# genglongling/EE274_ConvexCaldera_LLM_quantization

Hardware: AMD Instinct MI355X
Metric: weight matrices/sec (4096x4096, rank-128, Q=2-bit) + Frob err vs ref (higher is better)
Workload: dtype f32 (fp16 W in; fp32-grade split-fp16 MFMA products, fp64 small solves; int2 codes)

## Files before the change

### ee274_convexcaldera_llm_quantization_amd/_lib.py

```python
from __future__ import annotations

import contextlib
import ctypes
import os
import threading

import torch

from . import scratch

_HERE = os.path.dirname(os.path.abspath(__file__))
LIB_PATH = os.path.join(_HERE, "libcaldera_hip.so")

CQ_F32, CQ_F16, CQ_BF16, CQ_F64 = 0, 1, 2, 3
EPI_LINEAR, EPI_RESID, EPI_WERR = 0, 1, 2
CQ_EINVAL, CQ_EHIP, CQ_EWORKSPACE = -1, -2, -3

c_i64, c_int, c_float, c_double, c_size, c_vp = (ctypes.c_int64, ctypes.c_int, ctypes.c_float,
                                                 ctypes.c_double, ctypes.c_size_t, ctypes.c_void_p)


class GemmArgs(ctypes.Structure):
    _fields_ = [
        ("M", c_i64), ("N", c_i64), ("K", c_i64), ("batch", c_i64),
# ... 686 lines not shown
    M = MA if M is None else M
    N = Bh.shape[1]
    assert lda is None or (a_blocked and lda == MA and M <= MA)
    assert Bh.shape[2] == Kd and (C is None or C.shape == (Bt, M, N))
    for t in (Ah, Al, Bh, Bl, C, P, D, out_h, out_l):
        assert t is None or t.is_contiguous()
    for t in (out_h, out_l):
        assert t is None or t.numel() >= Bt * M * N, "gemm_x3: split output buffer too small"
    g = X3Args()
    g.M, g.N, g.K, g.batch = M, N, Kd, Bt
    g.Ah, g.Al, g.lda, g.stride_a = Ah.data_ptr(), Al.data_ptr(), (MA if a_blocked else Kd), MA * Kd
    g.Bh, g.Bl, g.ldb, g.stride_b = Bh.data_ptr(), (Bl.data_ptr() if Bl is not None else None), (
        N if b_blocked else Kd), N * Kd
    g.inv_scale = inv_scale.data_ptr()
    g.C, g.ldc, g.stride_c = (C.data_ptr() if C is not None else None), N, M * N
    if P is not None:
        g.P, g.ldp, g.stride_p = P.data_ptr(), N, M * N
    if D is not None:
        g.D, g.ldd, g.stride_d = D.data_ptr(), N, M * N
    g.alpha_v = alpha_v.data_ptr() if alpha_v is not None else None
    g.beta_v = beta_v.data_ptr() if beta_v is not None else None
    g.gamma_v = gamma_v.data_ptr() if gamma_v is not None else None
    if out_h is not None and sym_bound is None:
        g.out_h, g.out_l, g.ldo, g.stride_o = out_h.data_ptr(), out_l.data_ptr(), N, M * N
        g.out_scale = out_scale
        g.overflow = overflow.data_ptr()
    g.tri = int(bool(tri))
    g.b_blocked = int(b_blocked)
    g.active = active.data_ptr() if active is not None else None
    g.a_blocked = int(a_blocked)
    g.o_blocked = int(bool(o_blocked))
    g.single = int(bool(single))
    g.b_exact = int(bool(b_exact))
    if colw is not None:
        assert colw.dtype == torch.float32 and colw.is_contiguous() and colw.shape[-1] == N
        g.colw, g.stride_colw = colw.data_ptr(), _wst(colw, Bt)
    if absmax_out is not None:
        assert absmax_out.numel() == Bt and absmax_out.element_size() == 4 and absmax_out.is_contiguous()
        absmax_out.zero_()
        g.absmax_out = absmax_out.data_ptr()
    if Ct is not None:
        _require_hip(Ct)
        assert C is not None and not tri and Ct.dtype == torch.float32 and Ct.is_contiguous() and Ct.shape == (Bt, N, M)
        g.Ct, g.stride_ct = Ct.data_ptr(), N * M
    tiles = -(-N // 384) * -(-M // 192) * Bt
    splittable = not tri and sym_bound is None and C is not None and N % 4 == 0
    if ksplit is None and not auto_split_k():
        ksplit = 1
    if ksplit is None:
        ks = min(Kd // 32 // 8, -(-512 // tiles)) if splittable and tiles < 256 and Kd >= 512 else 1
    else:
        ks = int(ksplit)
        assert ks == 1 or (splittable and ks <= Kd // 32), "gemm_x3: split-K not possible here"
    if ks > 1:
        g.ksplit = ks
        g.split_ws = scratch.get_flat("gemm_x3.split", ks * Bt * M * N, torch.float32, Ah.device).data_ptr()
    if sym_bound is not None:
        g.sym_out = 1
        g.out_bound, g.scale_out, g.inv_out = sym_bound.data_ptr(), scale_out.data_ptr(), inv_out.data_ptr()
        g.out_h, g.out_l, g.ldo, g.stride_o = out_h.data_ptr(), out_l.data_ptr(), N, M * N
        g.out_scale = out_scale
    _check(load().cq_gemm_x3(ctypes.byref(g), _stream(Ah.device)), "cq_gemm_x3")
    return C


def q_update_x3(W: torch.Tensor, L: torch.Tensor | None, R: torch.Tensor | None, bits: int, *, eps: float = 1e-8,
                codes=None, packed=None, scale=None, err_w=None, err_out=None, events=None, absmax_in=None,
                scale_hint=None, fallback_out=None):
    _require_hip(W, L, R, codes, packed, scale, err_w, err_out, scale_hint, fallback_out)
# ... 214 lines not shown
```

### ee274_convexcaldera_llm_quantization_amd/csrc/cq_x3.hip

```cpp
#include <type_traits>
#include <numeric>

#include "cq_x3.h"

namespace cq {

__device__ __forceinline__ float sym_split_scale(double bound) {
    int e = 0;
    if (bound > 0.0 && isfinite(bound)) frexp(bound, &e);
    return ldexpf(1.f, 14 - e);
}

constexpr int XG_BK = 32;

__device__ __forceinline__ int xg_swz(int row) { return (0x78 >> (2 * ((row >> 2) & 3))) & 3; }

__device__ __forceinline__ f16x8g xg_frag(const _Float16* img, int row, int chunk) {
    const int pc = chunk ^ xg_swz(row);
    return *reinterpret_cast<const f16x8g*>(img + row * XG_BK + pc * 8);
}

constexpr int XW_BM = 192, XW_BN = 384, XW_BK = 32;
constexpr int XW_THREADS = 768;
constexpr int XW_APART = XW_BM * XW_BK, XW_BPART = XW_BN * XW_BK;
// ... 467 lines not shown
                    for (int r = 0; r < 4; ++r)
                        if (col + r >= row && col + r < a.N) { Oh[o + r] = h[r]; Ol[o + r] = l[r]; }
                }
#pragma unroll
                for (int r = 0; r < 4; ++r) {
                    const int64_t c = col + r;
                    if (c > row && c < a.N) {
                        const int64_t om = (row >> 5) * (M * 32) + c * 32 + (row & 31);
                        Oh[om] = h[r];
                        Ol[om] = l[r];
                    }
                }
            }
        }
        return;
    }
    const float al_ = !live ? 0.f : a.alpha_v ? a.alpha_v[b] : 1.f;
    const float be_ = !live ? 0.f : a.beta_v ? a.beta_v[b] : 0.f;
    const float ga_ = !live ? 1.f : a.gamma_v ? a.gamma_v[b] : 0.f;
    bool ovf = false;
    uint32_t amx = 0u;
    auto al16 = [](const void* p) { return (reinterpret_cast<uintptr_t>(p) & 15) == 0; };
    auto al8 = [](const void* p) { return (reinterpret_cast<uintptr_t>(p) & 7) == 0; };
    const bool vec = (a.N & 3) == 0 && (a.ldc & 3) == 0 && (a.sc & 3) == 0 && al16(a.C) &&
                     (!a.P || ((a.ldp & 3) == 0 && (a.sp & 3) == 0 && al16(a.P))) &&
                     (!a.D || ((a.ldd & 3) == 0 && (a.sd & 3) == 0 && al16(a.D))) &&
                     (!a.Oh || ((a.o_blocked || (a.ldo & 3) == 0) && (a.so & 3) == 0 && al8(a.Oh) && al8(a.Ol)));
#pragma unroll
    for (int i = 0; i < 6; ++i) {
        const int64_t row = m0 + 96 * wm + 16 * i + l16;
        if (row >= a.M) continue;
#pragma unroll
        for (int j = 0; j < 4; ++j) {
            const int64_t col = n0 + 64 * wn + 16 * j + 4 * lq;
            if (col >= a.N) continue;
            float v[4];
#pragma unroll
            for (int r = 0; r < 4; ++r) v[r] = al_ * (acc[i][j][r] * sc);
            if (a.colw) {
                const float* cw = a.colw + b * a.scolw;
#pragma unroll
                for (int r = 0; r < 4; ++r)
                    if (col + r < a.N) v[r] *= cw[col + r];
            }
            if (vec) {
                if (a.P && be_ != 0.f) {
                    const float4 pv = *reinterpret_cast<const float4*>(a.P + b * a.sp + row * a.ldp + col);
                    v[0] += be_ * pv.x; v[1] += be_ * pv.y; v[2] += be_ * pv.z; v[3] += be_ * pv.w;
                }
                if (a.D && ga_ != 0.f) {
                    const float4 dv = *reinterpret_cast<const float4*>(a.D + b * a.sd + row * a.ldd + col);
                    v[0] += ga_ * dv.x; v[1] += ga_ * dv.y; v[2] += ga_ * dv.z; v[3] += ga_ * dv.w;
                }
                *reinterpret_cast<float4*>(a.C + b * a.sc + row * a.ldc + col) = make_float4(v[0], v[1], v[2], v[3]);
                if (a.Ct) {
#pragma unroll
                    for (int r = 0; r < 4; ++r) a.Ct[b * a.sct + (col + r) * a.M + row] = v[r];
                }
                if (a.absmax_out)
                    amx = max(amx, max(max(abs_bits(v[0]), abs_bits(v[1])), max(abs_bits(v[2]), abs_bits(v[3]))));
                if (a.Oh) {
                    _Float16 h[4], l[4];
#pragma unroll
                    for (int r = 0; r < 4; ++r) {
                        const float hs = v[r] * a.out_scale;
                        h[r] = (_Float16)hs;
                        l[r] = (_Float16)(hs - (float)h[r]);
                        ovf |= !(fabsf(hs) < 65504.f);
                    }
                    const int64_t o = b * a.so + (a.o_blocked ? (col >> 5) * (a.M * 32) + row * 32 + (col & 31)
                                                              : row * a.ldo + col);
                    *reinterpret_cast<uint2*>(a.Oh + o) = *reinterpret_cast<const uint2*>(h);
                    *reinterpret_cast<uint2*>(a.Ol + o) = *reinterpret_cast<const uint2*>(l);
                }
            } else {
#pragma unroll
                for (int r = 0; r < 4; ++r) {
                    const int64_t c = col + r;
                    if (c >= a.N) continue;
                    float w = v[r];
                    if (a.P && be_ != 0.f) w += be_ * a.P[b * a.sp + row * a.ldp + c];
                    if (a.D && ga_ != 0.f) w += ga_ * a.D[b * a.sd + row * a.ldd + c];
                    a.C[b * a.sc + row * a.ldc + c] = w;
                    if (a.Ct) a.Ct[b * a.sct + c * a.M + row] = w;
                    amx = max(amx, abs_bits(w));
                    if (a.Oh) {
                        const float hs = w * a.out_scale;
                        const _Float16 h = (_Float16)hs;
                        const int64_t o = b * a.so + (a.o_blocked ? (c >> 5) * (a.M * 32) + row * 32 + (c & 31)
                                                                  : row * a.ldo + c);
                        a.Oh[o] = h;
                        a.Ol[o] = (_Float16)(hs - (float)h);
                        ovf |= !(fabsf(hs) < 65504.f);
                    }
                }
            }
        }
    }
    if (ovf) atomicOr(a.overflow + b, 1);
    if (a.absmax_out) {
        amx = wave_max_u32(amx);
        if (lane == 0 && amx) atomicMax(a.absmax_out + b, amx);
    }
}


constexpr int XS_BM = 256, XS_BN = 256, XS_THREADS = 512;
constexpr int XS_APART = XS_BM * XW_BK, XS_BPART = XS_BN * XW_BK;
constexpr int XS_STAGE = 2 * XS_APART + 2 * XS_BPART;
constexpr size_t XS_LDS_BYTES = (size_t)2 * XS_STAGE * sizeof(_Float16);
constexpr int XS_PER_WAVE = (2 * XS_BM / 16 + 2 * XS_BN / 16) / (XS_THREADS / 64);
static_assert(XS_PER_WAVE == 8, "load split");

__device__ __forceinline__ void xs_plan(const X3K& a, int64_t m0, int64_t n0, int wid, int lane,
                                        uint32_t (&off)[XS_PER_WAVE]) {
// ... 98 lines not shown
    const int64_t nq = a.N / 4;
    const int64_t t = (int64_t)blockIdx.x * 256 + threadIdx.x;
    const int64_t b = blockIdx.y;
    const bool in = t < a.M * nq;
    uint32_t amx = 0u;
    if (in) {
    const int64_t row = t / nq, col = 4 * (t % nq);
    const bool live = !a.active || a.active[b];
    const float al_ = !live ? 0.f : a.alpha_v ? a.alpha_v[b] : 1.f;
    const float be_ = !live ? 0.f : a.beta_v ? a.beta_v[b] : 0.f;
    const float ga_ = !live ? 1.f : a.gamma_v ? a.gamma_v[b] : 0.f;
    float s[4] = {0.f, 0.f, 0.f, 0.f};
    for (int ks = 0; ks < a.ksplit; ++ks) {
        const float4 pv = *reinterpret_cast<const float4*>(a.part + ((ks * a.batch + b) * a.M + row) * a.N + col);
        s[0] += pv.x; s[1] += pv.y; s[2] += pv.z; s[3] += pv.w;
    }
    bool ovf = false;
#pragma unroll
    for (int r = 0; r < 4; ++r) {
        float w = al_ * s[r];
        if (a.colw) w *= a.colw[b * a.scolw + col + r];
        if (a.P && be_ != 0.f) w += be_ * a.P[b * a.sp + row * a.ldp + col + r];
        if (a.D && ga_ != 0.f) w += ga_ * a.D[b * a.sd + row * a.ldd + col + r];
        a.C[b * a.sc + row * a.ldc + col + r] = w;
        if (a.Ct) a.Ct[b * a.sct + (col + r) * a.M + row] = w;
        amx = max(amx, abs_bits(w));
        if (a.Oh) {
            const float hs = w * a.out_scale;
            const _Float16 h = (_Float16)hs;
            const int64_t c = col + r;
            const int64_t o = b * a.so + (a.o_blocked ? (c >> 5) * (a.M * 32) + row * 32 + (c & 31) : row * a.ldo + c);
            a.Oh[o] = h;
            a.Ol[o] = (_Float16)(hs - (float)h);
            ovf |= !(fabsf(hs) < 65504.f);
        }
    }
    if (ovf) atomicOr(a.overflow + b, 1);
    }
    if (a.absmax_out) {
        amx = wave_max_u32(amx);
        if ((threadIdx.x & 63) == 0 && amx) atomicMax(a.absmax_out + b, amx);
    }
}


template <int PASS, int BITS>
__global__ __launch_bounds__(XW_THREADS, 1) void q_update_x3_kernel(QUK q) {
    extern __shared__ __attribute__((aligned(16))) char qu_smem_raw[];
    _Float16* smem = reinterpret_cast<_Float16*>(qu_smem_raw);
    const X3K& a = q.x;
    const int64_t tiles = a.tiles_n * a.tiles_m;
    const int64_t total = tiles * a.batch;
    const int64_t orig = blockIdx.x;
    const int64_t qq = total / 8, r8 = total % 8, xcd = orig % 8;
    const int64_t lin = (xcd < r8 ? xcd * (qq + 1) : r8 * (qq + 1) + (xcd - r8) * qq) + orig / 8;
    const int64_t tile = lin % tiles;
// ... 723 lines not shown
#pragma unroll
        for (int u = 0; u < 2; ++u) {
            const int i = il + 32 * u;
            const int64_t orow = c0 + i, ocol = r0 + 8 * g;
            if (orow >= cols || ocol >= rows) continue;
            float v[8];
#pragma unroll
            for (int q = 0; q < 8; ++q) v[q] = tile[8 * g + q][i];
            if (Y) {
                float* yp = Y + ob + orow * rows + ocol;
                *reinterpret_cast<float4*>(yp) = make_float4(v[0], v[1], v[2], v[3]);
                *reinterpret_cast<float4*>(yp + 4) = make_float4(v[4], v[5], v[6], v[7]);
            }
            if (hi) {
                _Float16 h[8], l[8];
#pragma unroll
                for (int q = 0; q < 8; ++q) {
                    const float xs = v[q] * s;
                    h[q] = (_Float16)xs;
                    l[q] = (_Float16)(xs - (float)h[q]);
                }
                const int64_t o = blocked ? ob + (ocol >> 5) * cols * 32 + orow * 32 + (ocol & 31) : ob + orow * rows + ocol;
                *reinterpret_cast<uint4*>(hi + o) = *reinterpret_cast<const uint4*>(h);
                *reinterpret_cast<uint4*>(lo + o) = *reinterpret_cast<const uint4*>(l);
            }
        }
        return;
    }
    for (int i = ty; i < 64; i += 4) {
        const int64_t r = r0 + i, c = c0 + tx;
        tile[i][tx] = (r < rows && c < cols) ? Xb[r * cols + c] : 0.f;
    }
    __syncthreads();
    for (int i = ty; i < 64; i += 4) {
        const int64_t orow = c0 + i, ocol = r0 + tx;
        if (orow < cols && ocol < rows) {
            const float v = tile[tx][i];
            if (Y) Y[ob + orow * rows + ocol] = v;
            if (hi) {
                const float xs = v * s;
                const _Float16 h = (_Float16)xs;
                const int64_t o = blocked ? ob + (ocol >> 5) * cols * 32 + orow * 32 + (ocol & 31) : ob + orow * rows + ocol;
                hi[o] = h;
                lo[o] = (_Float16)(xs - (float)h);
            }
        }
    }
}


}

using namespace cq;

extern "C" {

int cq_sym_split_f16(const float* G, int64_t n, int64_t batch, int upper_only, int blocked, float x_scale,
                     uint16_t* Gh, uint16_t* Gl, float* scale_out, float* inv_scale_out, void* stream) {
    CQ_REQUIRE(G && Gh && Gl && scale_out && inv_scale_out, "cq_sym_split_f16: null pointer");
    CQ_REQUIRE(n > 0 && batch > 0 && (n * n) % 4 == 0, "cq_sym_split_f16: bad shape");
    CQ_REQUIRE(x_scale > 0.f, "cq_sym_split_f16: x_scale must be > 0");
    hipStream_t s = as_stream(stream);
    sym_scale_kernel<<<(unsigned)batch, 256, 0, s>>>(G, n, n, n * n, x_scale, scale_out, inv_scale_out);
    CQ_REQUIRE(!blocked || n % 32 == 0, "cq_sym_split_f16: blocked layout needs n % 32 == 0");
    if (upper_only || blocked) {
        CQ_REQUIRE(batch < 65536, "cq_sym_split_f16: batch too large");
        const unsigned t64 = (unsigned)ceil_div(n, 64);
// ... 31 lines not shown
int cq_split_f16(const float* X, int64_t n_per, int64_t batch, const float* scale_v, float scale, uint16_t* hi,
                 uint16_t* lo, int64_t blocked_ncols, void* stream) {
    CQ_REQUIRE(X && hi && lo, "cq_split_f16: null pointer");
    CQ_REQUIRE(n_per > 0 && batch > 0 && n_per % 4 == 0, "cq_split_f16: n_per must be a positive multiple of 4");
    CQ_REQUIRE(blocked_ncols == 0 || (blocked_ncols % 32 == 0 && n_per % blocked_ncols == 0),
               "cq_split_f16: blocked layout needs ncols % 32 == 0 dividing n_per");
    const int64_t tot4 = batch * n_per / 4;
    const unsigned grid = (unsigned)std::min<int64_t>(ceil_div(tot4, 256), 8192);
    if (blocked_ncols) {
        const int64_t rows = n_per / blocked_ncols;
        CQ_REQUIRE(batch < 65536, "cq_split_f16: batch too large");
        split_blocked_kernel<<<dim3((unsigned)ceil_div(rows, 4), (unsigned)batch), 256, 0, as_stream(stream)>>>(
            X, rows, blocked_ncols, scale_v, scale, reinterpret_cast<_Float16*>(hi), reinterpret_cast<_Float16*>(lo));
        return check_launch("cq_split_f16");
    }
    split_kernel<<<grid, 256, 0, as_stream(stream)>>>(X, n_per, scale_v, scale, reinterpret_cast<_Float16*>(hi),
                                                      reinterpret_cast<_Float16*>(lo), batch);
    return check_launch("cq_split_f16");
}

int cq_transpose_split(const float* X, int64_t rows, int64_t cols, int64_t batch, float* Y, uint16_t* hi,
                       uint16_t* lo, float scale, const float* scale_v, int blocked, void* stream) {
    CQ_REQUIRE(!blocked || rows % 32 == 0, "cq_transpose_split: blocked halves need rows % 32 == 0");
    CQ_REQUIRE(X && (Y || (hi && lo)), "cq_transpose_split: null pointer");
    CQ_REQUIRE(!hi == !lo, "cq_transpose_split: hi and lo go together");
    CQ_REQUIRE(rows > 0 && cols > 0 && batch > 0 && batch < 65536, "cq_transpose_split: bad shape");
    dim3 grid((unsigned)ceil_div(cols, 64), (unsigned)ceil_div(rows, 64), (unsigned)batch);
    auto al16 = [](const void* p) { return (reinterpret_cast<uintptr_t>(p) & 15) == 0; };
    const bool vec = rows % 8 == 0 && cols % 4 == 0 && al16(X) && (!Y || al16(Y)) && (!hi || (al16(hi) && al16(lo)));
    if (vec)
        transpose_split_kernel<true><<<grid, 256, 0, as_stream(stream)>>>(
            X, rows, cols, Y, reinterpret_cast<_Float16*>(hi), reinterpret_cast<_Float16*>(lo), scale, scale_v, blocked);
    else
        transpose_split_kernel<false><<<grid, 256, 0, as_stream(stream)>>>(
            X, rows, cols, Y, reinterpret_cast<_Float16*>(hi), reinterpret_cast<_Float16*>(lo), scale, scale_v, blocked);
    return check_launch("cq_transpose_split");
}


static int64_t qu_tiles(int64_t m, int64_t n) {
    return std::max(ceil_div(n, XW_BM) * ceil_div(m, XW_BN), ceil_div(m, XW_BM) * ceil_div(n, XW_BN));
}

static size_t qu_cand_geom(int64_t m, int64_t n, int64_t batch, int rpw, int nw, int64_t* regions_out,
                           int64_t* cap_out, int64_t* capa_out = nullptr) {
    const int64_t regions = ceil_div(m, (int64_t)rpw * nw) * nw, groups = (int64_t)rpw * n / 8;
    const bool big = m * n >= QP_BIG_NUMEL;
    const int64_t cap = ceil_div(groups * (big ? QP_CAPB_PERMILLE_BIG : QP_CAPB_PERMILLE_SMALL), (int64_t)1000);
    const int64_t capa = ceil_div(groups * (big ? QP_CAPA_PERMILLE_BIG : QP_CAPA_PERMILLE_SMALL), (int64_t)1000);
    if (regions_out) *regions_out = regions;
    if (cap_out) *cap_out = cap;
    if (capa_out) *capa_out = capa;
// ... 192 lines not shown
    const int64_t gy = std::max<int64_t>(1, std::min<int64_t>(m / 32, 16));
    dim3 grid((unsigned)(n / 64), (unsigned)gy, (unsigned)batch);
    hipStream_t s = as_stream(stream);
    double* part = sq_out ? reinterpret_cast<double*>(ws) : nullptr;
    auto h = [](uint16_t* p) { return reinterpret_cast<_Float16*>(p); };
#define CQ_RS(DT, B) residual_split_kernel<DT, B><<<grid, 256, 0, s>>>(Ws, packed, qscale, ycol, wmax, ycol_max, m, n, \
        res_out, Y_out, h(hi), h(lo), h(thi), h(tlo), scale_out, part, ycol_hi, ycol_hi_max, scale_hi_out, \
        ycol_stride, ycol_max_v, ycol_hi_max_v)
    const int bsel = packed ? bits : 2;
    if (dtype == CQ_F16) {
        switch (bsel) { case 2: CQ_RS(CQ_F16, 2); break; case 4: CQ_RS(CQ_F16, 4); break;
                        case 8: CQ_RS(CQ_F16, 8); break; case 32: CQ_RS(CQ_F16, 32); break; default: CQ_RS(CQ_F16, 16); }
    } else {
        switch (bsel) { case 2: CQ_RS(CQ_F32, 2); break; case 4: CQ_RS(CQ_F32, 4); break;
                        case 8: CQ_RS(CQ_F32, 8); break; case 32: CQ_RS(CQ_F32, 32); break; default: CQ_RS(CQ_F32, 16); }
    }
#undef CQ_RS
    if (sq_out) sum_tile_parts_kernel<<<(unsigned)batch, 64, 0, s>>>(part, gy * (n / 64), sq_out);
    return check_launch("cq_residual_split");
}

int cq_gemm_x3(const cq_x3_args* g, void* stream) {
    CQ_REQUIRE(g, "cq_gemm_x3: null args");
    CQ_REQUIRE(g->Ah && g->Al && g->Bh && (g->Bl || g->single || g->b_exact) && (g->C || g->sym_out) && g->inv_scale,
               "cq_gemm_x3: null operand");
    CQ_REQUIRE(!g->sym_out || (g->tri && g->out_h && g->out_l && g->out_bound && g->scale_out && g->inv_out &&
                               g->out_scale > 0.f && g->N % 32 == 0),
               "cq_gemm_x3: sym_out needs tri, out_h/out_l, out_bound, scale_out, inv_out, N % 32 == 0");
    CQ_REQUIRE(g->M > 0 && g->N > 0 && g->K > 0 && g->batch > 0, "cq_gemm_x3: bad shape");
    CQ_REQUIRE(g->K % XW_BK == 0, "cq_gemm_x3: K must be a multiple of 32");
    CQ_REQUIRE(g->lda % 8 == 0 && g->ldb % 8 == 0 && g->stride_a % 8 == 0 && g->stride_b % 8 == 0,
               "cq_gemm_x3: operand rows must be 16-byte aligned");
    CQ_REQUIRE((g->a_blocked ? g->lda >= g->M : g->lda >= g->K) && (g->b_blocked ? g->ldb >= g->N : g->ldb >= g->K) &&
                   g->ldc >= g->N,
               "cq_gemm_x3: leading dimension too small");
    CQ_REQUIRE(!g->out_h == !g->out_l, "cq_gemm_x3: out_h and out_l go together");
    CQ_REQUIRE(!g->out_h || g->sym_out || (g->overflow && g->out_scale > 0.f),
               "cq_gemm_x3: split output needs overflow flags");
    CQ_REQUIRE(!g->beta_v || g->P, "cq_gemm_x3: beta_v needs P");
    CQ_REQUIRE(!g->gamma_v || g->D, "cq_gemm_x3: gamma_v needs D");
    X3K a;
    a.M = g->M; a.N = g->N; a.K = g->K; a.batch = g->batch;
    a.Ah = reinterpret_cast<const _Float16*>(g->Ah); a.Al = reinterpret_cast<const _Float16*>(g->Al);
    a.lda = g->lda; a.sa = g->stride_a;
    a.Bh = reinterpret_cast<const _Float16*>(g->Bh); a.Bl = reinterpret_cast<const _Float16*>(g->Bl);
    a.ldb = g->ldb; a.sb = g->stride_b;
    a.inv_scale = g->inv_scale;
    a.C = g->C; a.ldc = g->ldc; a.sc = g->stride_c;
    a.P = g->P; a.ldp = g->ldp; a.sp = g->stride_p;
    a.D = g->D; a.ldd = g->ldd; a.sd = g->stride_d;
    a.alpha_v = g->alpha_v; a.beta_v = g->beta_v; a.gamma_v = g->gamma_v;
    a.Oh = reinterpret_cast<_Float16*>(g->out_h); a.Ol = reinterpret_cast<_Float16*>(g->out_l);
    a.ldo = g->ldo; a.so = g->stride_o; a.out_scale = g->out_scale;
    a.overflow = g->overflow;
    CQ_REQUIRE(!g->tri || (g->M == g->N && !g->P && !g->D && (!g->out_h || g->sym_out)),
               "cq_gemm_x3: tri needs a square plain product");
    a.single = g->single;
    a.colw = g->colw;
    a.scolw = g->stride_colw;
    a.absmax_out = g->absmax_out;
    a.Ct = g->Ct;
    a.sct = g->stride_ct;
    CQ_REQUIRE(!g->Ct || (!g->sym_out && !g->tri && g->C), "cq_gemm_x3: Ct needs a non-symmetric product with C");
    CQ_REQUIRE(!g->absmax_out || (!g->sym_out && !g->tri), "cq_gemm_x3: absmax_out needs a plain product");
    CQ_REQUIRE(!g->colw || (!g->sym_out && !g->tri), "cq_gemm_x3: colw needs a plain product");
    a.sym_out = g->sym_out;
    a.out_bound = g->out_bound;
    a.scale_out = g->scale_out;
    a.inv_out = g->inv_out;
    a.tri = g->tri;
    a.b_blocked = g->b_blocked;
    a.active = g->active;
    a.a_blocked = g->a_blocked;
    a.o_blocked = g->o_blocked;
    CQ_REQUIRE(!g->o_blocked || g->N % 32 == 0, "cq_gemm_x3: blocked split output needs N % 32 == 0");
    CQ_REQUIRE(!g->a_blocked || g->lda >= g->M, "cq_gemm_x3: blocked A needs lda = rows >= M");
    CQ_REQUIRE(!g->active || g->D, "cq_gemm_x3: active needs D (the pass-through value)");
    CQ_REQUIRE(!g->b_blocked || g->ldb >= g->N, "cq_gemm_x3: blocked B needs ldb = rows >= N");
    a.tiles_n = ceil_div(g->N, XW_BN);
    a.tiles_m = ceil_div(g->M, XW_BM);
    int64_t total = a.tiles_n * a.tiles_m * a.batch;
    a.tiles_live = 0;
    if (a.sym_out) {
        static_assert(XW_BN == 2 * XW_BM, "Gram tile enumeration");
        for (int64_t tm = 0; tm < a.tiles_m; ++tm) a.tiles_live += std::max<int64_t>(0, a.tiles_n - (tm >> 1));
        total = a.tiles_live * a.batch;
    }
    a.ksplit = g->ksplit > 1 ? g->ksplit : 1;
    a.part = g->split_ws;
    if (a.ksplit > 1) {
        CQ_REQUIRE(!a.tri && !a.sym_out && a.part && a.C && g->N % 4 == 0 && a.ksplit <= g->K / XW_BK,
                   "cq_gemm_x3: split-K needs a plain product with C, N % 4 == 0, split_ws, ksplit <= K / 32");
        total *= a.ksplit;
    }
    CQ_REQUIRE(total < (1ll << 31), "cq_gemm_x3: grid too large");
    const bool sq = !a.single && !g->b_exact && !a.tri && !a.sym_out && a.ksplit == 1 && !a.P && !a.D && !a.Oh && !a.Ct &&
                    !a.colw && !a.active && g->M % XS_BM == 0 && g->N % XS_BN == 0 && g->ldc % 4 == 0 &&
                    g->stride_c % 4 == 0 && (reinterpret_cast<uintptr_t>(g->C) & 15) == 0 &&
                    (double)(a.tiles_m * XW_BM) * (double)(a.tiles_n * XW_BN) > 1.15 * (double)g->M * (double)g->N;
    if (sq) {
        a.tiles_m = g->M / XS_BM;
        a.tiles_n = g->N / XS_BN;
        const int64_t tot = a.tiles_m * a.tiles_n * a.batch;
        CQ_REQUIRE(tot < (1ll << 31), "cq_gemm_x3: grid too large");
        gemm_x3s_kernel<<<(unsigned)tot, XS_THREADS, XS_LDS_BYTES, as_stream(stream)>>>(a);
        return check_launch("cq_gemm_x3");
    }
    if (a.single) gemm_x3v_kernel<1><<<(unsigned)total, XW_THREADS, XW_LDS_BYTES, as_stream(stream)>>>(a);
    else if (g->b_exact) gemm_x3v_kernel<2><<<(unsigned)total, XW_THREADS, XW_LDS_BYTES, as_stream(stream)>>>(a);
    else gemm_x3v_kernel<0><<<(unsigned)total, XW_THREADS, XW_LDS_BYTES, as_stream(stream)>>>(a);
    if (a.ksplit > 1)
        x3_splitk_epi_kernel<<<dim3((unsigned)ceil_div(g->M * (g->N / 4), 256), (unsigned)g->batch), 256, 0,
                               as_stream(stream)>>>(a);
    return check_launch("cq_gemm_x3");
}
// ... 3 lines not shown
```

### ee274_convexcaldera_llm_quantization_amd/solver.py

```python
from __future__ import annotations

import math
import warnings

import numpy as np
import torch

from . import _lib as K
from . import scratch
from .overlap import run_to_end



TRANSPOSED_OUT = True

class _EventProbe:

    def __init__(self):
        self.on = False
        self.pool = []
        self.used = 0
        self.meta = []
        self.ref = None

# ... 8 lines not shown
            self.ref.record()

    def start(self, flops, nbytes=0.0, kernel=""):
        if not self.on or self.used >= len(self.pool):
            return None
        ev = self.pool[self.used]
        self.used += 1
        ev[0].record()
        self.meta.append((flops, nbytes, kernel))
        return ev

    def stop(self, ev):
        if ev is not None:
            ev[1].record()

    def summary(self):
        if not self.used:
            return {"count": 0}
        torch.cuda.synchronize()
        pairs = self.pool[: self.used]
        ms = [a.elapsed_time(b) for a, b in pairs]
        groups = {}
        for t, (fl, nb, kn) in zip(ms, self.meta):
            g = groups.setdefault(kn, {"count": 0, "ms": 0.0, "flops_per_launch": fl, "bytes_per_launch": nb})
            g["count"] += 1
            g["ms"] += t
        for g in groups.values():
            g["avg_ms"] = g["ms"] / g["count"]
        top = max(groups, key=lambda k: groups[k]["ms"])
        g = groups[top]
        out = {"count": g["count"], "avg_ms": g["avg_ms"], "flops_per_launch": g["flops_per_launch"],
               "bytes_per_launch": g["bytes_per_launch"], "kernel": top, "kernels": groups}
        if self.ref is not None:
            iv = sorted((self.ref.elapsed_time(a), self.ref.elapsed_time(b)) for a, b in pairs)
            union, cur_s, cur_e = 0.0, None, None
            for s0, e0 in iv:
                if cur_e is None or s0 > cur_e:
                    if cur_e is not None:
                        union += cur_e - cur_s
                    cur_s, cur_e = s0, e0
                else:
                    cur_e = max(cur_e, e0)
            union += cur_e - cur_s
            out["aggregate"] = {"launches": len(iv), "bytes": float(sum(nb for _, nb, _ in self.meta)),
                                "busy_ms": union, "window_ms": iv[-1][1] - iv[0][0] if iv else 0.0}
        return out


EVENT_PROBE = _EventProbe()


# ... 198 lines not shown
        eye = None
        for _ in range(steps):
            out = self._free(X, *keep)
            M = K.gram_f64(X, X)
            if eye is None:
                eye = torch.eye(self.p, dtype=torch.float64, device=X.device)
            N = (1.5 * eye - 0.5 * M).float()
            K.gemm(X, N, C=out)
            X = out
        return X, None

    def _orth2(self, X, *keep, halves=False):
        if self.ns_second:
            return self._ns(X, *keep)
        return self._cholqr(X, *keep, halves=halves)

    def _rr(self, X, *keep, single=False, values_only=False):
        G = self._G
        Z = self._free(X, *keep)
        if self.x3:
            if self._halves_of is not X:
                K.transpose_split(X, hi=self._xh[0], lo=self._xl[0], scale=X3_SCALE, blocked=True)
            self._halves_of = None
            K.gemm_x3(self._xh[0], self._xl[0], self._Gh, self._Gl, self._ginv, self._xt[0], b_blocked=self._g_blocked,
                      a_blocked=True, single=single and self._x3f, Ct=Z if TRANSPOSED_OUT else None)
            if not TRANSPOSED_OUT:
                K.transpose_split(self._xt[0], out=Z)
        else:
            K.gemm(G, X, ta=True, C=Z)
        self.stats.matvecs += 1
        T = K.gram_f64(X, Z)
        if values_only and self.values_lanczos > 0 and self.p <= 512:
            ends = K.extreme_eigs(T, self.values_lanczos)
            theta = torch.full((self.B, self.p), math.nan, dtype=torch.float64, device=T.device)
            theta[:, 0] = ends[:, 0]
            theta[:, self.p - 1] = ends[:, 1]
            self._last_sw = torch.zeros(self.B, dtype=torch.int32, device=T.device)
            return theta, X, None
        if values_only:
            theta, _, _, sw = yield from self._eigh(T, self.jacobi_tol_values, want_vectors=False,
                                                    max_sweeps=self.jacobi_values_sweeps)
            self._last_sw = sw
            return theta, X, None
        theta, V32, _, sw = yield from self._eigh(T, self.jacobi_tol)
        self._last_sw = sw
        Xo = self._free(X, Z, *keep)
        K.gemm(X, V32, C=Xo)
        Zo = self._free(X, Z, Xo, *keep)
# ... 74 lines not shown
        X0 = self._free(X, *keep)
        X0.copy_(X)
        Y1 = self._free(X, X0, *keep)
        fl = 2.0 * self.k * self.k * self.p * self.B
        nb = float(self.B) * (4.0 * self.k * self.k + 16.0 * self.p * self.k)
        kn = "gemm_f32_kernel (fp32 G X, Chebyshev filter)"
        ev = EVENT_PROBE.start(fl, nb, kn)
        K.gemm(G, X0, ta=True, C=Y1, D=X0, alpha_v=coef[0, 0], gamma_v=coef[0, 2])
        EVENT_PROBE.stop(ev)
        self.stats.matvecs += 1
        prev, cur = X0, Y1
        for i in range(1, deg):
            ev = EVENT_PROBE.start(fl, nb, kn)
            K.gemm(G, cur, ta=True, C=prev, D=cur, alpha_v=coef[i, 0], beta_v=coef[i, 1], gamma_v=coef[i, 2])
            EVENT_PROBE.stop(ev)
            self.stats.matvecs += 1
            prev, cur = cur, prev
        return cur

    def _filter_x3(self, X, coef, single=False, keep=()):
        deg = coef.shape[0]
        xt, xh, xl = self._xt, self._xh, self._xl
        self._halves_of = None
        K.transpose_split(X, out=xt[0], hi=xh[0], lo=xl[0], scale=X3_SCALE, blocked=True)
        fl = 2.0 * self.k * self.k * self.p * self.B
        nb = float(self.B) * (4.0 * self.k * self.k + 20.0 * self.p * self.k)
        kn = "gemm_x3v_kernel<0> (split-fp16 G X, Chebyshev filter)"
        if single:
            nb = float(self.B) * (2.0 * self.k * self.k + 18.0 * self.p * self.k)
            kn = "gemm_x3v_kernel<1> (single fp16 product G X, Chebyshev filter)"
        probe = EVENT_PROBE.start
        out = self._free(X, *keep)
        ct = out if TRANSPOSED_OUT else None
        last = deg == 1
        ev = probe(fl, nb, kn)
        K.gemm_x3(xh[0], xl[0], self._Gh, self._Gl, self._ginv, xt[1], D=xt[0], alpha_v=coef[0, 0],
                  gamma_v=coef[0, 2], out_h=None if last else xh[1], out_l=None if last else xl[1],
                  out_scale=X3_SCALE, overflow=self._ovf, b_blocked=self._g_blocked, active=self._active,
                  a_blocked=True, o_blocked=True, single=single, Ct=ct if last else None)
        EVENT_PROBE.stop(ev)
        self.stats.matvecs += 1
        prev, cur = 0, 1
        for i in range(1, deg):
            last = i == deg - 1
            ev = probe(fl, nb, kn)
            K.gemm_x3(xh[cur], xl[cur], self._Gh, self._Gl, self._ginv, xt[prev], P=xt[prev], D=xt[cur],
                      alpha_v=coef[i, 0], beta_v=coef[i, 1], gamma_v=coef[i, 2],
                      out_h=None if last else xh[prev], out_l=None if last else xl[prev],
                      out_scale=X3_SCALE, overflow=self._ovf, b_blocked=self._g_blocked,
                      active=self._active, a_blocked=True, o_blocked=True, single=single,
                      Ct=ct if last else None)
            EVENT_PROBE.stop(ev)
            self.stats.matvecs += 1
            prev, cur = cur, prev
        if ct is None:
            K.transpose_split(xt[cur], out=out)
        return out

    def solve(self, Y: torch.Tensor, warm: bool = True):
        return run_to_end(self.solve_iter(Y, warm))

    def solve_iter(self, Y: torch.Tensor, warm: bool = True, y_split=None, gram=None):
        B, k, p = self.B, self.k, self.p
        dev = Y.device
        self.stats.calls += 1
        if self.direct:
            Gd = K.gram_f64(Y, Y, ta=True, tb=True) if self.left else K.gram_f64(Y, Y)
            theta, V32, _, _ = K.jacobi_eigh(Gd)
            return V32[:, :, : self.r], theta[:, : self.r]
        self._alloc(dev)
        self._g_upper_only = False
        self._Y = Y
        self._y_halves = None
        g_split = False
# ... 268 lines not shown
```

Baseline: 338.9.

## Skip redundant GEMM epilogue stores and restructure vectorized epilogue addressing

The split-fp16 GEMM can now run without a row-major C when only the transposed output Ct is needed, and without lo halves when the following product is single-precision fp16. The Chebyshev filter and the Rayleigh-Ritz product drop these writes, and transpose_split skips lo halves in single mode. The vectorized epilogue precomputes per-thread 32-bit offsets from tile corners and loads P/D per fragment, aiming to cut 64-bit address arithmetic. This adds a new size limit check on M and the leading dimensions, and leaves more nullable-pointer paths to keep correct.

```diff
diff --git a/ee274_convexcaldera_llm_quantization_amd/_lib.py b/ee274_convexcaldera_llm_quantization_amd/_lib.py
--- a/ee274_convexcaldera_llm_quantization_amd/_lib.py
+++ b/ee274_convexcaldera_llm_quantization_amd/_lib.py
@@ -732,7 +732,7 @@
     g.beta_v = beta_v.data_ptr() if beta_v is not None else None
     g.gamma_v = gamma_v.data_ptr() if gamma_v is not None else None
     if out_h is not None and sym_bound is None:
-        g.out_h, g.out_l, g.ldo, g.stride_o = out_h.data_ptr(), out_l.data_ptr(), N, M * N
+        g.out_h, g.out_l, g.ldo, g.stride_o = out_h.data_ptr(), (out_l.data_ptr() if out_l is not None else None), N, M * N
         g.out_scale = out_scale
         g.overflow = overflow.data_ptr()
     g.tri = int(bool(tri))
@@ -751,10 +751,10 @@
         g.absmax_out = absmax_out.data_ptr()
     if Ct is not None:
         _require_hip(Ct)
-        assert C is not None and not tri and Ct.dtype == torch.float32 and Ct.is_contiguous() and Ct.shape == (Bt, N, M)
+        assert not tri and Ct.dtype == torch.float32 and Ct.is_contiguous() and Ct.shape == (Bt, N, M)
         g.Ct, g.stride_ct = Ct.data_ptr(), N * M
     tiles = -(-N // 384) * -(-M // 192) * Bt
-    splittable = not tri and sym_bound is None and C is not None and N % 4 == 0
+    splittable = not tri and sym_bound is None and (C is not None or Ct is not None) and N % 4 == 0
     if ksplit is None and not auto_split_k():
         ksplit = 1
     if ksplit is None:
diff --git a/ee274_convexcaldera_llm_quantization_amd/csrc/cq_x3.hip b/ee274_convexcaldera_llm_quantization_amd/csrc/cq_x3.hip
--- a/ee274_convexcaldera_llm_quantization_amd/csrc/cq_x3.hip
+++ b/ee274_convexcaldera_llm_quantization_amd/csrc/cq_x3.hip
@@ -513,66 +513,97 @@
     uint32_t amx = 0u;
     auto al16 = [](const void* p) { return (reinterpret_cast<uintptr_t>(p) & 15) == 0; };
     auto al8 = [](const void* p) { return (reinterpret_cast<uintptr_t>(p) & 7) == 0; };
-    const bool vec = (a.N & 3) == 0 && (a.ldc & 3) == 0 && (a.sc & 3) == 0 && al16(a.C) &&
+    const bool vec = (a.N & 3) == 0 && (!a.C || ((a.ldc & 3) == 0 && (a.sc & 3) == 0 && al16(a.C))) &&
                      (!a.P || ((a.ldp & 3) == 0 && (a.sp & 3) == 0 && al16(a.P))) &&
                      (!a.D || ((a.ldd & 3) == 0 && (a.sd & 3) == 0 && al16(a.D))) &&
-                     (!a.Oh || ((a.o_blocked || (a.ldo & 3) == 0) && (a.so & 3) == 0 && al8(a.Oh) && al8(a.Ol)));
-#pragma unroll
-    for (int i = 0; i < 6; ++i) {
-        const int64_t row = m0 + 96 * wm + 16 * i + l16;
-        if (row >= a.M) continue;
-#pragma unroll
-        for (int j = 0; j < 4; ++j) {
-            const int64_t col = n0 + 64 * wn + 16 * j + 4 * lq;
-            if (col >= a.N) continue;
+                     (!a.Oh || ((a.o_blocked || (a.ldo & 3) == 0) && (a.so & 3) == 0 && al8(a.Oh) && (!a.Ol || al8(a.Ol))));
+    if (vec) {
+        const bool useP = a.P && be_ != 0.f, useD = a.D && ga_ != 0.f;
+        const int mr = (int)min<int64_t>(a.M - m0, XW_BM), nr = (int)min<int64_t>(a.N - n0, XW_BN);
+        const uint32_t lr = 96 * wm + l16, lc = 64 * wn + 4 * lq;
+        auto corner = [&](const void* p, int64_t sb_, int64_t ld, int esz) __attribute__((always_inline)) {
+            return p ? reinterpret_cast<const char*>(p) + (b * sb_ + m0 * ld + n0) * esz : nullptr;
+        };
+        const char* Pt = corner(a.P, a.sp, a.ldp, 4);
+        const char* Dt = corner(a.D, a.sd, a.ldd, 4);
+        char* Ct_ = const_cast<char*>(corner(a.C, a.sc, a.ldc, 4));
+        char* Tt = a.Ct ? reinterpret_cast<char*>(a.Ct + b * a.sct + n0 * a.M + m0) : nullptr;
+        const float* cwt = a.colw ? a.colw + b * a.scolw + n0 : nullptr;
+        const uint32_t vP = (lr * (uint32_t)a.ldp + lc) * 4u, vD = (lr * (uint32_t)a.ldd + lc) * 4u,
+                       vC = (lr * (uint32_t)a.ldc + lc) * 4u, vT = (lc * (uint32_t)a.M + lr) * 4u;
+        const int64_t oblk = a.M * 32;
+        const int64_t ocorner = b * a.so + (a.o_blocked ? (n0 >> 5) * oblk + m0 * 32 : m0 * a.ldo + n0);
+        const uint32_t vO = (a.o_blocked ? (uint32_t)(2 * wn) * (uint32_t)oblk + lr * 32u + 4u * lq
+                                         : lr * (uint32_t)a.ldo + lc) * 2u;
+        auto inside = [&](int q) __attribute__((always_inline)) {
+            return (int)lr < mr - 16 * (q >> 2) && (int)lc < nr - 16 * (q & 3);
+        };
+        auto fetch = [&](int q, float4& pv, float4& dv) __attribute__((always_inline)) {
+            if (!inside(q)) return;
+            const int i = q >> 2, j = q & 3;
+            if (useP) pv = *reinterpret_cast<const float4*>(Pt + (16 * i * a.ldp + 16 * j) * 4 + vP);
+            if (useD) dv = *reinterpret_cast<const float4*>(Dt + (16 * i * a.ldd + 16 * j) * 4 + vD);
+        };
+        auto finish = [&](int q, const float4& pv, const float4& dv) __attribute__((always_inline)) {
+            if (!inside(q)) return;
+            const int i = q >> 2, j = q & 3;
+            const f32x4v ac = acc[i][j];
             float v[4];
 #pragma unroll
-            for (int r = 0; r < 4; ++r) v[r] = al_ * (acc[i][j][r] * sc);
-            if (a.colw) {
-                const float* cw = a.colw + b * a.scolw;
-#pragma unroll
-                for (int r = 0; r < 4; ++r)
-                    if (col + r < a.N) v[r] *= cw[col + r];
-            }
-            if (vec) {
-                if (a.P && be_ != 0.f) {
-                    const float4 pv = *reinterpret_cast<const float4*>(a.P + b * a.sp + row * a.ldp + col);
-                    v[0] += be_ * pv.x; v[1] += be_ * pv.y; v[2] += be_ * pv.z; v[3] += be_ * pv.w;
+            for (int r = 0; r < 4; ++r) v[r] = al_ * (ac[r] * sc);
+            if (cwt) {
+#pragma unroll
+                for (int r = 0; r < 4; ++r) v[r] *= cwt[lc + (uint32_t)(16 * j + r)];
+            }
+            if (useP) { v[0] += be_ * pv.x; v[1] += be_ * pv.y; v[2] += be_ * pv.z; v[3] += be_ * pv.w; }
+            if (useD) { v[0] += ga_ * dv.x; v[1] += ga_ * dv.y; v[2] += ga_ * dv.z; v[3] += ga_ * dv.w; }
+            if (Ct_) *reinterpret_cast<float4*>(Ct_ + (16 * i * a.ldc + 16 * j) * 4 + vC) = make_float4(v[0], v[1], v[2], v[3]);
+            if (Tt) {
+#pragma unroll
+                for (int r = 0; r < 4; ++r) *reinterpret_cast<float*>(Tt + ((16 * j + r) * a.M + 16 * i) * 4 + vT) = v[r];
+            }
+            if (a.absmax_out)
+                amx = max(amx, max(max(abs_bits(v[0]), abs_bits(v[1])), max(abs_bits(v[2]), abs_bits(v[3]))));
+            if (a.Oh) {
+                _Float16 h[4], l[4];
+#pragma unroll
+                for (int r = 0; r < 4; ++r) {
+                    const float hs = v[r] * a.out_scale;
+                    h[r] = (_Float16)hs;
+                    l[r] = (_Float16)(hs - (float)h[r]);
+                    ovf |= !(fabsf(hs) < 65504.f);
                 }
-                if (a.D && ga_ != 0.f) {
-                    const float4 dv = *reinterpret_cast<const float4*>(a.D + b * a.sd + row * a.ldd + col);
-                    v[0] += ga_ * dv.x; v[1] += ga_ * dv.y; v[2] += ga_ * dv.z; v[3] += ga_ * dv.w;
-                }
-                *reinterpret_cast<float4*>(a.C + b * a.sc + row * a.ldc + col) = make_float4(v[0], v[1], v[2], v[3]);
-                if (a.Ct) {
-#pragma unroll
-                    for (int r = 0; r < 4; ++r) a.Ct[b * a.sct + (col + r) * a.M + row] = v[r];
-                }
-                if (a.absmax_out)
-                    amx = max(amx, max(max(abs_bits(v[0]), abs_bits(v[1])), max(abs_bits(v[2]), abs_bits(v[3]))));
-                if (a.Oh) {
-                    _Float16 h[4], l[4];
-#pragma unroll
-                    for (int r = 0; r < 4; ++r) {
-                        const float hs = v[r] * a.out_scale;
-                        h[r] = (_Float16)hs;
-                        l[r] = (_Float16)(hs - (float)h[r]);
-                        ovf |= !(fabsf(hs) < 65504.f);
-                    }
-                    const int64_t o = b * a.so + (a.o_blocked ? (col >> 5) * (a.M * 32) + row * 32 + (col & 31)
-                                                              : row * a.ldo + col);
-                    *reinterpret_cast<uint2*>(a.Oh + o) = *reinterpret_cast<const uint2*>(h);
-                    *reinterpret_cast<uint2*>(a.Ol + o) = *reinterpret_cast<const uint2*>(l);
-                }
-            } else {
+                const int64_t oi = ocorner + (a.o_blocked ? (j >> 1) * oblk + 16 * i * 32 + 16 * (j & 1)
+                                                          : 16 * i * a.ldo + 16 * j);
+                *reinterpret_cast<uint2*>(reinterpret_cast<char*>(a.Oh + oi) + vO) = *reinterpret_cast<const uint2*>(h);
+                if (a.Ol) *reinterpret_cast<uint2*>(reinterpret_cast<char*>(a.Ol + oi) + vO) = *reinterpret_cast<const uint2*>(l);
+            }
+        };
+#pragma unroll
+        for (int q = 0; q < 24; ++q) {
+            float4 pv = make_float4(0.f, 0.f, 0.f, 0.f), dv = pv;
+            fetch(q, pv, dv);
+            finish(q, pv, dv);
+        }
+    } else {
+#pragma unroll
+        for (int i = 0; i < 6; ++i) {
+            const int64_t row = m0 + 96 * wm + 16 * i + l16;
+            if (row >= a.M) continue;
+#pragma unroll
+            for (int j = 0; j < 4; ++j) {
+                const int64_t col = n0 + 64 * wn + 16 * j + 4 * lq;
+                if (col >= a.N) continue;
+                const float* cw = a.colw ? a.colw + b * a.scolw : nullptr;
 #pragma unroll
                 for (int r = 0; r < 4; ++r) {
                     const int64_t c = col + r;
                     if (c >= a.N) continue;
-                    float w = v[r];
+                    float w = al_ * (acc[i][j][r] * sc);
+                    if (cw) w *= cw[c];
                     if (a.P && be_ != 0.f) w += be_ * a.P[b * a.sp + row * a.ldp + c];
                     if (a.D && ga_ != 0.f) w += ga_ * a.D[b * a.sd + row * a.ldd + c];
-                    a.C[b * a.sc + row * a.ldc + c] = w;
+                    if (a.C) a.C[b * a.sc + row * a.ldc + c] = w;
                     if (a.Ct) a.Ct[b * a.sct + c * a.M + row] = w;
                     amx = max(amx, abs_bits(w));
                     if (a.Oh) {
@@ -581,7 +612,7 @@
                         const int64_t o = b * a.so + (a.o_blocked ? (c >> 5) * (a.M * 32) + row * 32 + (c & 31)
                                                                   : row * a.ldo + c);
                         a.Oh[o] = h;
-                        a.Ol[o] = (_Float16)(hs - (float)h);
+                        if (a.Ol) a.Ol[o] = (_Float16)(hs - (float)h);
                         ovf |= !(fabsf(hs) < 65504.f);
                     }
                 }
@@ -726,7 +757,7 @@
         if (a.colw) w *= a.colw[b * a.scolw + col + r];
         if (a.P && be_ != 0.f) w += be_ * a.P[b * a.sp + row * a.ldp + col + r];
         if (a.D && ga_ != 0.f) w += ga_ * a.D[b * a.sd + row * a.ldd + col + r];
-        a.C[b * a.sc + row * a.ldc + col + r] = w;
+        if (a.C) a.C[b * a.sc + row * a.ldc + col + r] = w;
         if (a.Ct) a.Ct[b * a.sct + (col + r) * a.M + row] = w;
         amx = max(amx, abs_bits(w));
         if (a.Oh) {
@@ -735,7 +766,7 @@
             const int64_t c = col + r;
             const int64_t o = b * a.so + (a.o_blocked ? (c >> 5) * (a.M * 32) + row * 32 + (c & 31) : row * a.ldo + c);
             a.Oh[o] = h;
-            a.Ol[o] = (_Float16)(hs - (float)h);
+            if (a.Ol) a.Ol[o] = (_Float16)(hs - (float)h);
             ovf |= !(fabsf(hs) < 65504.f);
         }
     }
@@ -1505,7 +1536,7 @@
                 }
                 const int64_t o = blocked ? ob + (ocol >> 5) * cols * 32 + orow * 32 + (ocol & 31) : ob + orow * rows + ocol;
                 *reinterpret_cast<uint4*>(hi + o) = *reinterpret_cast<const uint4*>(h);
-                *reinterpret_cast<uint4*>(lo + o) = *reinterpret_cast<const uint4*>(l);
+                if (lo) *reinterpret_cast<uint4*>(lo + o) = *reinterpret_cast<const uint4*>(l);
             }
         }
         return;
@@ -1525,7 +1556,7 @@
                 const _Float16 h = (_Float16)xs;
                 const int64_t o = blocked ? ob + (ocol >> 5) * cols * 32 + orow * 32 + (ocol & 31) : ob + orow * rows + ocol;
                 hi[o] = h;
-                lo[o] = (_Float16)(xs - (float)h);
+                if (lo) lo[o] = (_Float16)(xs - (float)h);
             }
         }
     }
@@ -1603,12 +1634,12 @@
 int cq_transpose_split(const float* X, int64_t rows, int64_t cols, int64_t batch, float* Y, uint16_t* hi,
                        uint16_t* lo, float scale, const float* scale_v, int blocked, void* stream) {
     CQ_REQUIRE(!blocked || rows % 32 == 0, "cq_transpose_split: blocked halves need rows % 32 == 0");
-    CQ_REQUIRE(X && (Y || (hi && lo)), "cq_transpose_split: null pointer");
-    CQ_REQUIRE(!hi == !lo, "cq_transpose_split: hi and lo go together");
+    CQ_REQUIRE(X && (Y || hi), "cq_transpose_split: null pointer");
+    CQ_REQUIRE(hi || !lo, "cq_transpose_split: lo needs hi (hi alone: the operand of a single product)");
     CQ_REQUIRE(rows > 0 && cols > 0 && batch > 0 && batch < 65536, "cq_transpose_split: bad shape");
     dim3 grid((unsigned)ceil_div(cols, 64), (unsigned)ceil_div(rows, 64), (unsigned)batch);
     auto al16 = [](const void* p) { return (reinterpret_cast<uintptr_t>(p) & 15) == 0; };
-    const bool vec = rows % 8 == 0 && cols % 4 == 0 && al16(X) && (!Y || al16(Y)) && (!hi || (al16(hi) && al16(lo)));
+    const bool vec = rows % 8 == 0 && cols % 4 == 0 && al16(X) && (!Y || al16(Y)) && (!hi || al16(hi)) && (!lo || al16(lo));
     if (vec)
         transpose_split_kernel<true><<<grid, 256, 0, as_stream(stream)>>>(
             X, rows, cols, Y, reinterpret_cast<_Float16*>(hi), reinterpret_cast<_Float16*>(lo), scale, scale_v, blocked);
@@ -1847,7 +1878,7 @@
 
 int cq_gemm_x3(const cq_x3_args* g, void* stream) {
     CQ_REQUIRE(g, "cq_gemm_x3: null args");
-    CQ_REQUIRE(g->Ah && g->Al && g->Bh && (g->Bl || g->single || g->b_exact) && (g->C || g->sym_out) && g->inv_scale,
+    CQ_REQUIRE(g->Ah && g->Al && g->Bh && (g->Bl || g->single || g->b_exact) && (g->C || g->sym_out || g->Ct) && g->inv_scale,
                "cq_gemm_x3: null operand");
     CQ_REQUIRE(!g->sym_out || (g->tri && g->out_h && g->out_l && g->out_bound && g->scale_out && g->inv_out &&
                                g->out_scale > 0.f && g->N % 32 == 0),
@@ -1857,9 +1888,11 @@
     CQ_REQUIRE(g->lda % 8 == 0 && g->ldb % 8 == 0 && g->stride_a % 8 == 0 && g->stride_b % 8 == 0,
                "cq_gemm_x3: operand rows must be 16-byte aligned");
     CQ_REQUIRE((g->a_blocked ? g->lda >= g->M : g->lda >= g->K) && (g->b_blocked ? g->ldb >= g->N : g->ldb >= g->K) &&
-                   g->ldc >= g->N,
+                   (!g->C || g->ldc >= g->N),
                "cq_gemm_x3: leading dimension too small");
-    CQ_REQUIRE(!g->out_h == !g->out_l, "cq_gemm_x3: out_h and out_l go together");
+    CQ_REQUIRE(g->out_h || !g->out_l, "cq_gemm_x3: out_l needs out_h (out_h alone: hi halves only)");
+    CQ_REQUIRE(g->M <= (1 << 21) && g->ldc <= (1 << 22) && g->ldp <= (1 << 22) && g->ldd <= (1 << 22) && g->ldo <= (1 << 22),
+               "cq_gemm_x3: M above 2^21 or a leading dimension above 2^22");
     CQ_REQUIRE(!g->out_h || g->sym_out || (g->overflow && g->out_scale > 0.f),
                "cq_gemm_x3: split output needs overflow flags");
     CQ_REQUIRE(!g->beta_v || g->P, "cq_gemm_x3: beta_v needs P");
@@ -1886,7 +1919,7 @@
     a.absmax_out = g->absmax_out;
     a.Ct = g->Ct;
     a.sct = g->stride_ct;
-    CQ_REQUIRE(!g->Ct || (!g->sym_out && !g->tri && g->C), "cq_gemm_x3: Ct needs a non-symmetric product with C");
+    CQ_REQUIRE(!g->Ct || (!g->sym_out && !g->tri), "cq_gemm_x3: Ct needs a non-symmetric product");
     CQ_REQUIRE(!g->absmax_out || (!g->sym_out && !g->tri), "cq_gemm_x3: absmax_out needs a plain product");
     CQ_REQUIRE(!g->colw || (!g->sym_out && !g->tri), "cq_gemm_x3: colw needs a plain product");
     a.sym_out = g->sym_out;
@@ -1914,8 +1947,8 @@
     a.ksplit = g->ksplit > 1 ? g->ksplit : 1;
     a.part = g->split_ws;
     if (a.ksplit > 1) {
-        CQ_REQUIRE(!a.tri && !a.sym_out && a.part && a.C && g->N % 4 == 0 && a.ksplit <= g->K / XW_BK,
-                   "cq_gemm_x3: split-K needs a plain product with C, N % 4 == 0, split_ws, ksplit <= K / 32");
+        CQ_REQUIRE(!a.tri && !a.sym_out && a.part && (a.C || a.Ct) && g->N % 4 == 0 && a.ksplit <= g->K / XW_BK,
+                   "cq_gemm_x3: split-K needs a plain product with C or Ct, N % 4 == 0, split_ws, ksplit <= K / 32");
         total *= a.ksplit;
     }
     CQ_REQUIRE(total < (1ll << 31), "cq_gemm_x3: grid too large");
diff --git a/ee274_convexcaldera_llm_quantization_amd/solver.py b/ee274_convexcaldera_llm_quantization_amd/solver.py
--- a/ee274_convexcaldera_llm_quantization_amd/solver.py
+++ b/ee274_convexcaldera_llm_quantization_amd/solver.py
@@ -54,11 +54,13 @@
         ms = [a.elapsed_time(b) for a, b in pairs]
         groups = {}
         for t, (fl, nb, kn) in zip(ms, self.meta):
-            g = groups.setdefault(kn, {"count": 0, "ms": 0.0, "flops_per_launch": fl, "bytes_per_launch": nb})
+            g = groups.setdefault(kn, {"count": 0, "ms": 0.0, "flops_per_launch": fl, "bytes_per_launch": 0.0})
             g["count"] += 1
             g["ms"] += t
+            g["bytes_per_launch"] += nb
         for g in groups.values():
             g["avg_ms"] = g["ms"] / g["count"]
+            g["bytes_per_launch"] /= g["count"]
         top = max(groups, key=lambda k: groups[k]["ms"])
         g = groups[top]
         out = {"count": g["count"], "avg_ms": g["avg_ms"], "flops_per_launch": g["flops_per_launch"],
@@ -303,8 +305,9 @@
             if self._halves_of is not X:
                 K.transpose_split(X, hi=self._xh[0], lo=self._xl[0], scale=X3_SCALE, blocked=True)
             self._halves_of = None
-            K.gemm_x3(self._xh[0], self._xl[0], self._Gh, self._Gl, self._ginv, self._xt[0], b_blocked=self._g_blocked,
-                      a_blocked=True, single=single and self._x3f, Ct=Z if TRANSPOSED_OUT else None)
+            K.gemm_x3(self._xh[0], self._xl[0], self._Gh, self._Gl, self._ginv, None if TRANSPOSED_OUT else self._xt[0],
+                      b_blocked=self._g_blocked, a_blocked=True, single=single and self._x3f,
+                      Ct=Z if TRANSPOSED_OUT else None)
             if not TRANSPOSED_OUT:
                 K.transpose_split(self._xt[0], out=Z)
         else:
@@ -425,34 +428,42 @@
         deg = coef.shape[0]
         xt, xh, xl = self._xt, self._xh, self._xl
         self._halves_of = None
-        K.transpose_split(X, out=xt[0], hi=xh[0], lo=xl[0], scale=X3_SCALE, blocked=True)
+        K.transpose_split(X, out=xt[0], hi=xh[0], lo=None if single else xl[0], scale=X3_SCALE, blocked=True)
         fl = 2.0 * self.k * self.k * self.p * self.B
-        nb = float(self.B) * (4.0 * self.k * self.k + 20.0 * self.p * self.k)
-        kn = "gemm_x3v_kernel<0> (split-fp16 G X, Chebyshev filter)"
-        if single:
-            nb = float(self.B) * (2.0 * self.k * self.k + 18.0 * self.p * self.k)
-            kn = "gemm_x3v_kernel<1> (single fp16 product G X, Chebyshev filter)"
+        pk = float(self.p) * self.k
+        gb = (2.0 if single else 4.0) * self.k * self.k
+        nb_mid = float(self.B) * (gb + (16.0 if single else 20.0) * pk)
+        kn = ("gemm_x3v_kernel<1> (single fp16 product G X, Chebyshev filter)" if single
+              else "gemm_x3v_kernel<0> (split-fp16 G X, Chebyshev filter)")
         probe = EVENT_PROBE.start
         out = self._free(X, *keep)
         ct = out if TRANSPOSED_OUT else None
+        nb_last = float(self.B) * (gb + (14.0 if single else 16.0) * pk)
+
+        def outputs(last, c):
+            if not last:
+                return dict(C=xt[c], out_h=xh[c], out_l=None if single else xl[c], Ct=None)
+            return dict(C=xt[c] if ct is None else None, out_h=None, out_l=None, Ct=ct)
+
         last = deg == 1
-        ev = probe(fl, nb, kn)
-        K.gemm_x3(xh[0], xl[0], self._Gh, self._Gl, self._ginv, xt[1], D=xt[0], alpha_v=coef[0, 0],
-                  gamma_v=coef[0, 2], out_h=None if last else xh[1], out_l=None if last else xl[1],
+        o = outputs(last, 1)
+        ev = probe(fl, nb_last if last else nb_mid, kn)
+        K.gemm_x3(xh[0], xl[0], self._Gh, self._Gl, self._ginv, o["C"], D=xt[0], alpha_v=coef[0, 0],
+                  gamma_v=coef[0, 2], out_h=o["out_h"], out_l=o["out_l"],
                   out_scale=X3_SCALE, overflow=self._ovf, b_blocked=self._g_blocked, active=self._active,
-                  a_blocked=True, o_blocked=True, single=single, Ct=ct if last else None)
+                  a_blocked=True, o_blocked=True, single=single, Ct=o["Ct"])
         EVENT_PROBE.stop(ev)
         self.stats.matvecs += 1
         prev, cur = 0, 1
         for i in range(1, deg):
             last = i == deg - 1
-            ev = probe(fl, nb, kn)
-            K.gemm_x3(xh[cur], xl[cur], self._Gh, self._Gl, self._ginv, xt[prev], P=xt[prev], D=xt[cur],
+            o = outputs(last, prev)
+            ev = probe(fl, nb_last if last else nb_mid, kn)
+            K.gemm_x3(xh[cur], xl[cur], self._Gh, self._Gl, self._ginv, o["C"], P=xt[prev], D=xt[cur],
                       alpha_v=coef[i, 0], beta_v=coef[i, 1], gamma_v=coef[i, 2],
-                      out_h=None if last else xh[prev], out_l=None if last else xl[prev],
+                      out_h=o["out_h"], out_l=o["out_l"],
                       out_scale=X3_SCALE, overflow=self._ovf, b_blocked=self._g_blocked,
-                      active=self._active, a_blocked=True, o_blocked=True, single=single,
-                      Ct=ct if last else None)
+                      active=self._active, a_blocked=True, o_blocked=True, single=single, Ct=o["Ct"])
             EVENT_PROBE.stop(ev)
             self.stats.matvecs += 1
             prev, cur = cur, prev
```

New measurement: 345.8, median of 6. +2.0%, better.
